# Vinmwaura/Quantized-Autoregression-Image-Generator

Measured on AMD Instinct MI355X. Metric: image-tokens/sec at 1/2/4/8 GPUs; BMU argmin GB/s vs HBM peak, higher is better.
Workload: dtype f32; 1 GPU; BASELINE configs[1]: BMU (K=512; LR patch 32, HR patch 2) + base decoder-only Transformer train step, 32x32x4 latents (128x128 images), 257-token sequences, window 256; batch_per_gpu=64, global_batch=64, seq_len=256, in_dim=512, hidden_dim=2048, heads=64, dec_layers=7, enc_layers=0, params=78226440, parallelism=dp1, launch=eager stream launches

## Files before the change

include/qarig.h:

```cpp
#ifndef QARIG_H
#define QARIG_H

#include <stddef.h>
#include <stdint.h>

#ifdef __cplusplus
extern "C" {
#endif

#define QARIG_OK 0
#define QARIG_ERR_ARG -1
#define QARIG_ERR_LAUNCH -2
#define QARIG_ERR_WORKSPACE -3

#define QARIG_ACT_NONE 0
#define QARIG_ACT_SILU 1
#define QARIG_ACT_TANH 2
#define QARIG_ACT_SIGMOID 3

int qarig_version(void);
const char* qarig_target_arch(void);
int qarig_last_error(char* buf, size_t n);
int qarig_set_option(const char* name, int value);

// ... 129 lines not shown

int qarig_decode_decide(int* ctl, int N, int NB, int beam_width, int draws, float* comb,
                        const int64_t* chunk, float* best_p, int64_t* best_chunk, int* take, void* stream);

int qarig_decode_rows(const int* ctl, float* kv, float* staged, const int* take, int layers2, int N,
                      int NB, int H, int R, int d, int max_len, int restore, void* stream);

int qarig_decode_cache_fill(const float* k, const float* v, int64_t ld, int64_t batch_stride, float* kv,
                            int images, int beams, int H, int d, int P1, int max_len, void* stream);

int qarig_decode_commit(int* ctl, int N, int NB, int beam_width, const int64_t* best_chunk,
                        int64_t* tokens, int64_t ldt, int64_t* ids, void* stream);

int qarig_decode_advance(int* ctl, int beam_width, void* stream);


int qarig_window_step_supported(int R, int window, int D, int H);

int qarig_window_assemble(const int64_t* ring, int64_t ldr, const int* ctl, int R, int W1, int Wp, int D,
                          int V, const float* table, const float* pe, int P, int pos_off, float* x,
                          int* rowmap, int* last_map, int* bad_flag, void* stream);

int qarig_window_attention(const float* q, const float* k, const float* v, int R, int H, int d, int n_keys,
                           int rows, int64_t batch_stride, const float* o_mul, int64_t ldmul, float* o,
                           void* stream);

int qarig_window_append(int* ctl, const int64_t* ids, int64_t* ring, int B, int64_t ldr, int* bad_flag,
                        void* stream);

size_t qarig_colsum_workspace_bytes(int M, int N);
int qarig_colsum_f32(const float* X, int64_t ldx, int M, int N, float* out, int accumulate,
                     void* workspace, size_t ws_bytes, void* stream);


int qarig_patchify_fwd(const float* image, int N, int C, int H, int W, int pH, int pW,
                       float* patches, void* stream);
int qarig_unpatchify_fwd(const float* patches, int N, int C, int H, int W, int pH, int pW,
                         float* image, void* stream);

int qarig_codebook_gather_image(const int64_t* ids, int N, int C, int H, int W, int pH, int pW,
                                const float* codebook, int K, float* image, int* bad_flag,
                                void* stream);

int qarig_gather_rows(const int64_t* ids, int64_t R, int D, int K, const float* table, float* out,
                      int* bad_flag, void* stream);

int qarig_som_weights_fwd(const int64_t* bmu, int64_t R, int K, float two_var, float* g,
                          void* stream);

int qarig_som_band(const float* in, int K, int D, float two_var, int reach, float* out, void* stream);

int qarig_index_histogram(const int64_t* ids, int64_t n, int K, int64_t* counts, int* bad_flag,
                          void* stream);


int qarig_posemb_fwd(const float* pos, int R, int D, const float* freq, float* out, void* stream);

int qarig_assemble_tokens(const int64_t* lr, int S_lr, const int64_t* hr, int S_hr, int N, int base,
                          int k_lr, int k_hr, const int64_t* offs, int W, int64_t* hr_in,
                          int64_t* hr_tg, int64_t* pos, int* bad_flag, void* stream);

int qarig_embedding_fwd(const int64_t* ids, int M, int S, int D, int V, const float* table,
                        const float* pe, float* out, int* bad_flag, void* stream);
int qarig_embedding_bwd(const int64_t* ids, int M, int D, int V, const float* dy, float* dtable,
                        void* stream);

int qarig_layernorm_fwd(const float* x, int M, int D, float eps, const float* gamma,
                        const float* beta, const float* scale, const float* shift,
                        const int* mod_idx, float* y, float* mean, float* rstd, void* stream);
int qarig_layernorm_bwd(const float* dy, const float* x, const float* mean, const float* rstd,
                        const float* gamma, const float* scale, const int* mod_idx, int M, int D,
                        float* dx, float* dy_xhat, const float* dx_add, void* stream);

int qarig_rowmap_build(const int* idx, int M, int P, int* counts, int* offsets, int* rows,
                       int* bad_flag, void* stream);
int qarig_segment_sum(const float* src, const int* offsets, const int* rows, int P, int D,
                      float* out, void* stream);
int qarig_mul_rows_fwd(const float* a, const float* tab, const int* idx, float* y, int M, int D,
                       void* stream);
int qarig_mul_rows_bwd(const float* dy, const float* a, const float* tab, const int* idx, float* da,
                       float* db_tok, int M, int D, void* stream);

int qarig_attention_fwd(const float* q, const float* k, const float* v, int N, int Sq, int Sk,
                        int H, int d, int causal, float sqrt_d, float* o, float* lse,
                        void* stream);
int qarig_attention_bwd(const float* q, const float* k, const float* v, const float* o,
                        const float* dO, const float* lse, int N, int Sq, int Sk, int H, int d,
                        int causal, float sqrt_d, float* dq, float* dk, float* dv, float* delta,
                        void* stream);

int qarig_attention_lp_fwd(const float* q, const float* k, const float* v, int N, int Sq, int Sk, int H,
                           int d, int causal, float sqrt_d, float* o, float* lse, void* stream);
int qarig_attention_lp_bwd(const float* q, const float* k, const float* v, const float* o,
                           const float* dO, const float* lse, int N, int Sq, int Sk, int H, int d,
                           int causal, float sqrt_d, float* dq, float* dk, float* dv, float* delta,
                           void* stream);

int qarig_attention_decode(const float* q, const float* k_new, const float* v_new, float* kcache,
                           float* vcache, int B, int H, int d, int len, const int* len_dev,
                           int max_len, int64_t batch_stride, float sqrt_d, const float* o_mul,
                           float* o, void* stream);

int qarig_cross_entropy_fwd(const float* logits, const int64_t* target, int M, int C, float* loss,
                            float* dlogits, float* row_ws, int* bad_flag, void* stream);

size_t qarig_mse_workspace_bytes(void);
int qarig_mse_fwd(const float* pred, const float* target, int64_t n, float* loss, float* dpred,
                  float* part_ws, void* stream);

int qarig_adam_step(float* p, const float* g, float* m, float* v, int64_t n, float beta1,
                    float beta2, float eps, float step_size, float bc2_sqrt, float grad_scale,
                    const float* dev_step, void* shadow_bf16, void* stream);

int qarig_adam_ema_step(float* p, const float* g, float* m, float* v, float* ema, int64_t n, float beta1,
// ... 50 lines not shown
```

quantized-autoregression-image-generator_amd/csrc/condtable.hip:

```cpp
#include "qarig_common.h"

namespace qarig {

__global__ __launch_bounds__(256) void rowmap_count_kernel(const int* __restrict__ idx, int M, int P,
                                                           int* __restrict__ cnt,
                                                           int* __restrict__ bad) {
    const int p = blockIdx.x;
    int c = 0;
    for (int r = threadIdx.x; r < M; r += 256) {
        const int v = idx[r];
        c += v == p;
        if (p == 0 && (v < 0 || v >= P)) atomicExch(bad, 1);
    }
    __shared__ int part[4];
    c = (int)wave_sum((float)c);
    if ((threadIdx.x & 63) == 0) part[threadIdx.x >> 6] = c;
    __syncthreads();
    if (threadIdx.x == 0) cnt[p] = part[0] + part[1] + part[2] + part[3];
}

__global__ __launch_bounds__(256) void rowmap_scan_kernel(const int* __restrict__ cnt, int P,
                                                          int* __restrict__ offsets) {
    __shared__ int carry;
    __shared__ int buf[256];
// ... 69 lines not shown
            *reinterpret_cast<float4*>(out + (int64_t)p * D + c) = r;
        }
    }
}

__global__ void mul_rows_kernel(const float* __restrict__ a, const float* __restrict__ tab,
                                const int* __restrict__ idx, float* __restrict__ y, int M, int D4) {
    const int64_t total = (int64_t)M * D4;
    for (int64_t i = (int64_t)blockIdx.x * blockDim.x + threadIdx.x; i < total;
         i += (int64_t)gridDim.x * blockDim.x) {
        const int r = (int)(i / D4), c4 = (int)(i - (int64_t)r * D4);
        const float4 av = reinterpret_cast<const float4*>(a)[i];
        const float4 bv = reinterpret_cast<const float4*>(tab)[(int64_t)idx[r] * D4 + c4];
        reinterpret_cast<float4*>(y)[i] = make_float4(av.x * bv.x, av.y * bv.y, av.z * bv.z, av.w * bv.w);
    }
}

__global__ void mul_rows_bwd_kernel(const float* __restrict__ dy, const float* __restrict__ a,
                                    const float* __restrict__ tab, const int* __restrict__ idx,
                                    float* __restrict__ da, float* __restrict__ db_tok, int M,
                                    int D4) {
    const int64_t total = (int64_t)M * D4;
    for (int64_t i = (int64_t)blockIdx.x * blockDim.x + threadIdx.x; i < total;
         i += (int64_t)gridDim.x * blockDim.x) {
        const int r = (int)(i / D4), c4 = (int)(i - (int64_t)r * D4);
        const float4 d = reinterpret_cast<const float4*>(dy)[i];
        const float4 av = reinterpret_cast<const float4*>(a)[i];
        const float4 bv = reinterpret_cast<const float4*>(tab)[(int64_t)idx[r] * D4 + c4];
        reinterpret_cast<float4*>(da)[i] = make_float4(d.x * bv.x, d.y * bv.y, d.z * bv.z, d.w * bv.w);
        reinterpret_cast<float4*>(db_tok)[i] = make_float4(d.x * av.x, d.y * av.y, d.z * av.z, d.w * av.w);
    }
}

}

using namespace qarig;

static dim3 ct_grid(int64_t total) {
    int64_t b = (total + 255) / 256;
    return dim3((unsigned)(b > 8192 ? 8192 : (b < 1 ? 1 : b)));
}

extern "C" int qarig_rowmap_build(const int* idx, int M, int P, int* counts, int* offsets, int* rows,
                                  int* bad_flag, void* stream) {
    QARIG_CHECK_ARG(idx && counts && offsets && rows && bad_flag && M > 0 && P > 0,
                    "rowmap_build: bad arguments");
    QARIG_CHECK_DIMS("rowmap_build", M);
    QARIG_CHECK_DIMS("rowmap_build", P);
    hipStream_t st = (hipStream_t)stream;
    hipLaunchKernelGGL(rowmap_count_kernel, dim3(P), dim3(256), 0, st, idx, M, P, counts, bad_flag);
    QARIG_CHECK_LAUNCH("rowmap count");
    hipLaunchKernelGGL(rowmap_scan_kernel, dim3(1), dim3(256), 0, st, counts, P, offsets);
    QARIG_CHECK_LAUNCH("rowmap scan");
    hipLaunchKernelGGL(rowmap_fill_kernel, dim3(P), dim3(64), 0, st, idx, M, offsets, rows);
    QARIG_CHECK_LAUNCH("rowmap fill");
    return QARIG_OK;
}

extern "C" int qarig_segment_sum(const float* src, const int* offsets, const int* rows, int P, int D,
                                 float* out, void* stream) {
    QARIG_CHECK_ARG(src && offsets && rows && out && P > 0 && D > 0 && D % 4 == 0 &&
                        ((((uintptr_t)src | (uintptr_t)out)) & 15) == 0,
                    "segment_sum: bad arguments (D %% 4 == 0, 16-B aligned)");
    QARIG_CHECK_DIMS("segment_sum", P, D);
    hipLaunchKernelGGL(segment_sum_kernel, dim3(P, (D + 511) / 512), dim3(512), 0,
                       (hipStream_t)stream, src, offsets, rows, D, out);
    QARIG_CHECK_LAUNCH("segment_sum");
    return QARIG_OK;
}

extern "C" int qarig_mul_rows_fwd(const float* a, const float* tab, const int* idx, float* y, int M,
                                  int D, void* stream) {
    QARIG_CHECK_ARG(a && tab && idx && y && M > 0 && D > 0 && D % 4 == 0 &&
                        ((((uintptr_t)a | (uintptr_t)tab | (uintptr_t)y)) & 15) == 0,
                    "mul_rows_fwd: bad arguments (D %% 4 == 0, 16-B aligned)");
    QARIG_CHECK_DIMS("mul_rows_fwd", M, D);
    hipLaunchKernelGGL(mul_rows_kernel, ct_grid((int64_t)M * (D / 4)), dim3(256), 0,
                       (hipStream_t)stream, a, tab, idx, y, M, D / 4);
    QARIG_CHECK_LAUNCH("mul_rows_fwd");
    return QARIG_OK;
}

extern "C" int qarig_mul_rows_bwd(const float* dy, const float* a, const float* tab, const int* idx,
                                  float* da, float* db_tok, int M, int D, void* stream) {
    QARIG_CHECK_ARG(dy && a && tab && idx && da && db_tok && M > 0 && D > 0 && D % 4 == 0 &&
                        ((((uintptr_t)dy | (uintptr_t)a | (uintptr_t)tab | (uintptr_t)da |
                           (uintptr_t)db_tok)) & 15) == 0,
                    "mul_rows_bwd: bad arguments (D %% 4 == 0, 16-B aligned)");
    QARIG_CHECK_DIMS("mul_rows_bwd", M, D);
    hipLaunchKernelGGL(mul_rows_bwd_kernel, ct_grid((int64_t)M * (D / 4)), dim3(256), 0,
                       (hipStream_t)stream, dy, a, tab, idx, da, db_tok, M, D / 4);
    QARIG_CHECK_LAUNCH("mul_rows_bwd");
    return QARIG_OK;
}
```

quantized-autoregression-image-generator_amd/csrc/gemm.hip:

```cpp
#include <stdlib.h>

#include "qarig_common.h"
#include "gemm_epilogue.h"
#include "ring_common.h"

namespace qarig {

struct RowSumHook {
    float rs;
    bool on;
    int tid;
    __device__ __forceinline__ void operator()(const float* ta, const float*) {
        if (on) {
#pragma unroll
            for (int kk = 0; kk < BK; ++kk) rs += ta[kk * LDT + tid];
        }
    }
};

template <class SA, class SB, bool FAST>
__global__ __launch_bounds__(NTHREADS, 2) void gemm_kernel(SA sa, SB sb, GemmEpilogue ep, int M,
                                                           int N, int K, int tiles_n, int splitk,
                                                           float* slabs, int vec_epi) {
    __shared__ __attribute__((aligned(16))) float lds[GEMM_LDS_FLOATS];
// ... 385 lines not shown
__global__ void slab_reduce_kernel(const float* __restrict__ slabs, float* __restrict__ out,
                                   int64_t ldc, int M, int N, int nslab, int accumulate) {
    const int64_t total = (int64_t)M * N;
    for (int64_t i = (int64_t)blockIdx.x * blockDim.x + threadIdx.x; i < total;
         i += (int64_t)gridDim.x * blockDim.x) {
        float s = 0.0f;
        for (int z = 0; z < nslab; ++z) s += slabs[(int64_t)z * total + i];
        const int64_t row = i / N, col = i - row * N;
        out[row * ldc + col] = accumulate ? out[row * ldc + col] + s : s;
    }
}

__global__ void slab_reduce_rowsum_kernel(const float* __restrict__ slabs, float* __restrict__ out,
                                          int64_t ldc, int M, int N, int nslab, int accumulate, int nb,
                                          const float* __restrict__ rs_part, float* __restrict__ rs_out) {
    if ((int)blockIdx.x >= nb) {
        const int m = ((int)blockIdx.x - nb) * blockDim.x + threadIdx.x;
        if (m < M) {
            float s = 0.0f;
            for (int z = 0; z < nslab; ++z) s += rs_part[(int64_t)z * M + m];
            rs_out[m] = accumulate ? rs_out[m] + s : s;
        }
        return;
    }
    const int64_t total = (int64_t)M * N;
    for (int64_t i = (int64_t)blockIdx.x * blockDim.x + threadIdx.x; i < total; i += (int64_t)nb * blockDim.x) {
        float s = 0.0f;
        for (int z = 0; z < nslab; ++z) s += slabs[(int64_t)z * total + i];
        const int64_t row = i / N, col = i - row * N;
        out[row * ldc + col] = accumulate ? out[row * ldc + col] + s : s;
    }
}

__global__ void slab_reduce_epilogue_kernel(const float* __restrict__ slabs, GemmEpilogue ep, int M,
                                            int N, int nslab) {
    const int64_t total = (int64_t)M * N;
    for (int64_t i = (int64_t)blockIdx.x * blockDim.x + threadIdx.x; i < total;
         i += (int64_t)gridDim.x * blockDim.x) {
        float t = 0.0f;
        for (int z = 0; z < nslab; ++z) t += slabs[(int64_t)z * total + i];
        const int64_t row = i / N, col = i - row * N;
        if (ep.bias) t += ep.bias[col];
        if (ep.residual) t += ep.residual[row * ep.ldr + col];
        if (ep.preact) ep.preact[row * ep.ldp + col] = t;
        float y = act_fwd(t, ep.act);
        if (ep.gradz) y *= act_grad(ep.gradz[row * ep.ldz + col], ep.gact);
        ep.C[row * ep.ldc + col] = y;
    }
}

static inline int colsum_rows(int M) { return M >= 32768 ? 512 : (M >= 8192 ? 128 : 32); }
__global__ __launch_bounds__(256) void colsum_partial_kernel(const float* __restrict__ X,
                                                             int64_t ldx, int M, int N,
                                                             float* __restrict__ part, int rows) {
    __shared__ float red[4][64];
    const int cx = threadIdx.x & 63, ry = threadIdx.x >> 6;
    const int col = blockIdx.x * 64 + cx;
    const int r0 = blockIdx.y * rows;
    const int r1 = min(M, r0 + rows);
    float s = 0.0f;
    if (col < N)
        for (int r = r0 + ry; r < r1; r += 4) s += X[(int64_t)r * ldx + col];
    red[ry][cx] = s;
    __syncthreads();
    if (ry == 0 && col < N)
        part[(int64_t)blockIdx.y * N + col] = ((red[0][cx] + red[1][cx]) + red[2][cx]) + red[3][cx];
// ... 303 lines not shown
                               M, N, K, tiles_n, splitk, slabs);
    } else if (pf && fast && vec_epi && !(a_rowsum && a_kcontig) && !(!a_kcontig && b_kcontig)) {
        const int xs = (splitk % 8 == 0 && g_qarig_opt.gemm_xcd_splits != 0) ? 1 : 0;
        const dim3 pgrid = xs ? dim3(grid.x * splitk, 1, 1) : grid;
        if (a_kcontig && b_kcontig)
            hipLaunchKernelGGL((gemm_dma_pf_kernel<true, true>), pgrid, block, 0, st, A, lda, B, ldb, ep, M,
                               N, K, tiles_n, splitk, slabs, xs);
        else if (a_kcontig)
            hipLaunchKernelGGL((gemm_dma_pf_kernel<true, false>), pgrid, block, 0, st, A, lda, B, ldb, ep, M,
                               N, K, tiles_n, splitk, slabs, xs);
        else
            hipLaunchKernelGGL((gemm_dma_pf_kernel<false, false>), pgrid, block, 0, st, A, lda, B, ldb, ep,
                               M, N, K, tiles_n, splitk, slabs, xs);
    } else {
#define QARIG_LAUNCH_GEMM(TA, TB)                                                              \
    do {                                                                                       \
        TA sa{A, lda, M, K, 1.0f, va};                                                         \
        TB sb{B, ldb, N, K, 1.0f, vb};                                                         \
        if (fast)                                                                              \
            hipLaunchKernelGGL((gemm_kernel<TA, TB, true>), grid, block, 0, st, sa, sb, ep, M, \
                               N, K, tiles_n, splitk, slabs, vec_epi);                         \
        else                                                                                   \
            hipLaunchKernelGGL((gemm_kernel<TA, TB, false>), grid, block, 0, st, sa, sb, ep, M,\
                               N, K, tiles_n, splitk, slabs, 0);                               \
    } while (0)
    if (a_kcontig && b_kcontig) QARIG_LAUNCH_GEMM(SrcKContig, SrcKContig);
    else if (a_kcontig && !b_kcontig) QARIG_LAUNCH_GEMM(SrcKContig, SrcXContig);
    else if (!a_kcontig && !b_kcontig) QARIG_LAUNCH_GEMM(SrcXContig, SrcXContig);
    else QARIG_LAUNCH_GEMM(SrcXContig, SrcKContig);
#undef QARIG_LAUNCH_GEMM
    }
    QARIG_CHECK_LAUNCH("gemm");
    if (a_rowsum && splitk > 1 && plain) {
        const int64_t total = (int64_t)M * N;
        int blocks = (int)((total + 255) / 256);
        if (blocks > 2048) blocks = 2048;
        hipLaunchKernelGGL(slab_reduce_rowsum_kernel, dim3(blocks + (M + 255) / 256), dim3(256), 0, st, slabs, C,
                           ldc, M, N, splitk, accumulate, blocks, rs_part, a_rowsum);
        QARIG_CHECK_LAUNCH("gemm slab + rowsum reduce");
        return QARIG_OK;
    }
    if (a_rowsum) {
        hipLaunchKernelGGL(slab_reduce_kernel, dim3((M + 255) / 256), dim3(256), 0, st, rs_part,
                           a_rowsum, (int64_t)M, 1, M, splitk, accumulate);
        QARIG_CHECK_LAUNCH("gemm rowsum reduce");
    }
    if (splitk > 1) {
        const int64_t total = (int64_t)M * N;
        int blocks = (int)((total + 255) / 256);
        if (blocks > 2048) blocks = 2048;
        if (plain)
            hipLaunchKernelGGL(slab_reduce_kernel, dim3(blocks), dim3(256), 0, st, slabs, C, ldc, M, N,
                               splitk, accumulate);
        else
            hipLaunchKernelGGL(slab_reduce_epilogue_kernel, dim3(blocks), dim3(256), 0, st, slabs, ep,
                               M, N, splitk);
        QARIG_CHECK_LAUNCH("gemm slab reduce");
    }
    return QARIG_OK;
}

extern "C" int qarig_slab_reduce_f32(const float* slabs, float* out, int64_t ldc, int M, int N,
                                     int nslab, int accumulate, void* stream) {
    const int64_t total = (int64_t)M * N;
    int blocks = (int)((total + 255) / 256);
    if (blocks > 2048) blocks = 2048;
    hipLaunchKernelGGL(slab_reduce_kernel, dim3(blocks), dim3(256), 0, (hipStream_t)stream, slabs, out,
                       ldc, M, N, nslab, accumulate);
    QARIG_CHECK_LAUNCH("slab reduce");
    return QARIG_OK;
}

extern "C" size_t qarig_colsum_workspace_bytes(int M, int N) {
    if (M < 1 || N < 1 || M > (1 << 30)) return 0;
    const int rows = colsum_rows(M);
    const int chunks = (M + rows - 1) / rows;
    return (size_t)chunks * N * sizeof(float);
}

extern "C" int qarig_colsum_f32(const float* X, int64_t ldx, int M, int N, float* out,
                                int accumulate, void* workspace, size_t ws_bytes, void* stream) {
    QARIG_CHECK_ARG(X && out && M > 0 && N > 0, "colsum: bad arguments");
    QARIG_CHECK_DIMS("colsum", M, N);
    if (!workspace || ws_bytes < qarig_colsum_workspace_bytes(M, N)) {
        qarig_set_error("colsum: workspace too small");
        return QARIG_ERR_WORKSPACE;
    }
    const int rows = colsum_rows(M);
    const int chunks = (M + rows - 1) / rows;
    hipStream_t st = (hipStream_t)stream;
    float* part = (float*)workspace;
    hipLaunchKernelGGL(colsum_partial_kernel, dim3((N + 63) / 64, chunks), dim3(256), 0, st, X, ldx,
                       M, N, part, rows);
    QARIG_CHECK_LAUNCH("colsum partial");
    int blocks = (N + 255) / 256;
    hipLaunchKernelGGL(slab_reduce_kernel, dim3(blocks), dim3(256), 0, st, part, out, (int64_t)N, 1,
                       N, chunks, accumulate);
    QARIG_CHECK_LAUNCH("colsum reduce");
    return QARIG_OK;
}

// ... 171 lines not shown
```

quantized-autoregression-image-generator_amd/qarig/_lib.py:

```python
import ctypes
import os
from ctypes import c_int, c_int64, c_size_t, c_void_p, c_float, c_char_p

import torch

_HERE = os.path.dirname(os.path.abspath(__file__))
LIB_PATH = os.path.join(os.path.dirname(_HERE), "lib",
                        os.environ.get("QARIG_LIB", "libqarig_hip.so"))

P = c_void_p
I = c_int
L = c_int64
Z = c_size_t
F = c_float

SIGNATURES = {
    "qarig_version": (I, []),
    "qarig_target_arch": (c_char_p, []),
    "qarig_last_error": (I, [c_char_p, Z]),
    "qarig_set_option": (I, [c_char_p, I]),
    "qarig_bmu_workspace_bytes": (Z, [L, I]),
    "qarig_bmu_fwd": (I, [P, I, I, I, I, I, I, P, I, I, P, P, Z, P]),
    "qarig_bmu_fwd_prepared": (I, [P, I, I, I, I, I, I, P, I, I, P, P, Z, P, P]),
    "qarig_bmu_fwd_coarse": (I, [P, I, I, I, I, I, I, P, I, I, P, P, P, P]),
# ... 16 lines not shown
                          P]),
    "qarig_gemm_f8_supported": (I, [I, I, I]),
    "qarig_cast_fp8": (I, [P, L, P, P, P, P, P]),
    "qarig_gemm_f8": (I, [P, L, P, L, P, P, P, L, I, I, I, P, P, L, P, L, I, P, L, P, L, P]),
    "qarig_mx_quant_workspace_bytes": (Z, [I, I]),
    "qarig_mx_quant": (I, [P, L, I, I, I, P, P, P, P, P, I, P, Z, P]),
    "qarig_gemm_mx_supported": (I, [I, I, I, I]),
    "qarig_gemm_mx_workspace_bytes": (Z, [I, I, I]),
    "qarig_gemm_mx": (I, [P, L, P, L, P, L, P, L, P, L, I, I, I, P, P, L, P, L, I, P, L, I, I, I, I, P, L, P, L,
                          P, Z, P]),
    "qarig_cast_colsum_workspace_bytes": (Z, [I, I]),
    "qarig_cast_colsum": (I, [P, L, I, I, I, P, P, I, P, Z, P]),
    "qarig_cast_bf16": (I, [P, P, L, P]),
    "qarig_cast_transpose_bf16": (I, [P, L, I, I, P, P]),
    "qarig_colsum_workspace_bytes": (Z, [I, I]),
    "qarig_colsum_f32": (I, [P, L, I, I, P, I, P, Z, P]),
    "qarig_patchify_fwd": (I, [P, I, I, I, I, I, I, P, P]),
    "qarig_unpatchify_fwd": (I, [P, I, I, I, I, I, I, P, P]),
    "qarig_codebook_gather_image": (I, [P, I, I, I, I, I, I, P, I, P, P, P]),
    "qarig_gather_rows": (I, [P, L, I, I, P, P, P, P]),
    "qarig_som_weights_fwd": (I, [P, L, I, F, P, P]),
    "qarig_som_band": (I, [P, I, I, F, I, P, P]),
    "qarig_index_histogram": (I, [P, L, I, P, P, P]),
    "qarig_posemb_fwd": (I, [P, I, I, P, P, P]),
    "qarig_assemble_tokens": (I, [P, I, P, I, I, I, I, I, P, I, P, P, P, P, P]),
    "qarig_embedding_fwd": (I, [P, I, I, I, I, P, P, P, P, P]),
    "qarig_embedding_bwd": (I, [P, I, I, I, P, P, P]),
    "qarig_layernorm_fwd": (I, [P, I, I, F, P, P, P, P, P, P, P, P, P]),
    "qarig_layernorm_bwd": (I, [P, P, P, P, P, P, P, I, I, P, P, P, P]),
    "qarig_rowmap_build": (I, [P, I, I, P, P, P, P, P]),
    "qarig_segment_sum": (I, [P, P, P, I, I, P, P]),
    "qarig_mul_rows_fwd": (I, [P, P, P, P, I, I, P]),
    "qarig_mul_rows_bwd": (I, [P, P, P, P, P, P, I, I, P]),
    "qarig_attention_fwd": (I, [P, P, P, I, I, I, I, I, I, F, P, P, P]),
    "qarig_attention_lp_fwd": (I, [P, P, P, I, I, I, I, I, I, F, P, P, P]),
    "qarig_attention_lp_bwd": (I, [P, P, P, P, P, P, I, I, I, I, I, I, F, P, P, P, P, P]),
    "qarig_attention_decode": (I, [P, P, P, P, P, I, I, I, I, P, I, L, F, P, P, P]),
    "qarig_gemm_grouped_skinny_f32": (I, [P, L, L, P, L, L, P, L, L, P, L, I, I, I, I, I, P]),
    "qarig_gemm_skinny_ln_f32": (I, [P, L, F, P, P, P, P, L, P, L, L, P, L, L, P, L, P, L, I, I, I, I, I, P]),
    "qarig_decode_linear_supported": (I, [I, I, I, I]),
    "qarig_decode_linear_f32": (I, [P, L, L, F, P, P, P, P, L, P, L, L, P, L, P, L, P, L, P, L, L, I, I, I, I, I,
                                    P]),
    "qarig_decode_linear_bf16w": (I, [P, L, L, F, P, P, P, P, L, P, L, L, P, L, P, L, P, L, P, L, L, I, I, I, I, I,
                                      P]),
    "qarig_decode_embed": (I, [P, I, I, I, P, P, P, I, I, P, L, P, P, P, P]),
    "qarig_decode_attention_keys_per_pass": (ctypes.c_uint, [I]),
    "qarig_decode_attention": (I, [P, P, P, P, P, I, I, I, I, P, I, L, L, L, F, P, L, P, P]),
    "qarig_decode_sample": (I, [P, L, I, I, F, I, I, L, P, P, P, I, I, I, I, I, P, P, P, P, P]),
    "qarig_decode_sample_filtered": (I, [P, L, I, I, F, I, I, L, P, P, P, I, I, I, I, I, P, P, P, P, I, F, P]),
    "qarig_decode_decide": (I, [P, I, I, I, I, P, P, P, P, P, P]),
    "qarig_decode_rows": (I, [P, P, P, P, I, I, I, I, I, I, I, I, P]),
    "qarig_decode_cache_fill": (I, [P, P, L, L, P, I, I, I, I, I, I, P]),
    "qarig_decode_commit": (I, [P, I, I, I, P, P, L, P, P]),
    "qarig_decode_advance": (I, [P, I, P]),
    "qarig_window_step_supported": (I, [I, I, I, I]),
    "qarig_window_assemble": (I, [P, L, P, I, I, I, I, I, P, P, I, I, P, P, P, P, P]),
    "qarig_window_attention": (I, [P, P, P, I, I, I, I, I, L, P, L, P, P]),
    "qarig_window_append": (I, [P, P, P, I, L, P, P]),
    "qarig_attention_bwd": (I, [P, P, P, P, P, P, I, I, I, I, I, I, F, P, P, P, P, P]),
    "qarig_cross_entropy_fwd": (I, [P, P, I, I, P, P, P, P, P]),
    "qarig_mse_workspace_bytes": (Z, []),
    "qarig_mse_fwd": (I, [P, P, L, P, P, P, P]),
    "qarig_adam_step": (I, [P, P, P, P, L, F, F, F, F, F, F, P, P, P]),
    "qarig_adam_ema_step": (I, [P, P, P, P, P, L, F, F, F, F, F, F, F, P, P, P]),
    "qarig_swap_f32": (I, [P, P, L, P]),
    "qarig_mul_fwd": (I, [P, P, P, L, P]),
# ... 131 lines not shown
```

quantized-autoregression-image-generator_amd/qarig/functional.py:

```python
import os

import torch

from . import ops
from ._lib import f32c, require_cuda


def _2d(t):
    return t.reshape(-1, t.shape[-1])


FUSED_GRAD_ACCUMULATE = True


def _grad_slot(param):
    if not FUSED_GRAD_ACCUMULATE or not isinstance(param, torch.nn.Parameter):
        return None
    g = param.grad
    if g is None or not g.is_contiguous() or g.dtype != torch.float32 or g.shape != param.shape:
        return None
    return g


def _report_done(param):
# ... 787 lines not shown
        return tuple(grads)

    @staticmethod
    def backward(ctx, *douts):
        if ctx.tiled:
            return _TableProjections._backward_tiled(ctx, douts)
        tab, W = ctx.saved_tensors
        G, D, _ = W.shape
        P = tab.shape[0]
        cols = [f32c(d) if d is not None else torch.zeros((P, D), dtype=torch.float32, device=tab.device)
                for d in douts]
        dcat = torch.cat(cols, dim=1)
        W2 = W.reshape(G * D, D)
        dtab = ops.gemm(dcat, W2, a_kcontig=True, b_kcontig=False) if ctx.needs_input_grad[0] else None
        dW = ops.gemm(dcat, tab, a_kcontig=False, b_kcontig=False,
                      splitk=ops.pick_splitk(G * D, D, P)).reshape(G, D, D)
        db = ops.colsum(dcat).reshape(G, D)
        grads = [dtab]
        wparams, bparams = ctx.params[0::2], ctx.params[1::2]
        wslots = [_grad_slot(p) for p in wparams]
        bslots = [_grad_slot(p) for p in bparams]
        if all(s is not None for s in wslots) and all(s is not None for s in bslots):
            torch._foreach_add_(wslots, list(dW.unbind(0)))
            torch._foreach_add_(bslots, list(db.unbind(0)))
            for p in ctx.params:
                _report_done(p)
            grads += [None] * len(ctx.params)
        else:
            for g in range(G):
                grads += [dW[g], db[g]]
        return tuple(grads)


class _LayerNormModTable(torch.autograd.Function):

    @staticmethod
    def forward(ctx, x, scale_tab, shift_tab, idx, offsets, rows, eps, with_skip=False):
        require_cuda(x, scale_tab, shift_tab)
        x2 = _2d(f32c(x))
        st = f32c(scale_tab)
        y, mean, rstd = ops.layernorm_fwd(x2, scale=st, shift=f32c(shift_tab), eps=eps, mod_idx=idx)
        ctx.save_for_backward(x2, st, mean, rstd, idx, offsets, rows)
        ctx.shape = x.shape
        ctx.set_materialize_grads(False)
        return _with_skip(y.reshape(x.shape), x, with_skip)

    @staticmethod
    def backward(ctx, dy, dskip=None):
        x2, st, mean, rstd, idx, offsets, rows = ctx.saved_tensors
        dy2, add = _skip_grads(dy, dskip, x2)
        dx, dscale_tok = ops.layernorm_bwd(dy2, x2, mean, rstd, scale=st, want_dy_xhat=True,
                                           mod_idx=idx, dx_add=add)
        dscale = ops.segment_sum(dscale_tok, offsets, rows)
        dshift = ops.segment_sum(dy2, offsets, rows)
        return dx.reshape(ctx.shape), dscale, dshift, None, None, None, None, None


def layernorm_mod_table(x, scale_tab, shift_tab, cond, eps=1e-5, with_skip=False):
    if _no_grad():
        require_cuda(x, scale_tab, shift_tab)
        y = ops.layernorm_fwd(_2d(f32c(x)), scale=f32c(scale_tab), shift=f32c(shift_tab), eps=eps,
                              mod_idx=cond.idx)[0].reshape(x.shape)
        return (y, x) if with_skip else y
    return _LayerNormModTable.apply(x, scale_tab, shift_tab, cond.idx, cond.offsets, cond.rows, eps, with_skip)


class _MulTable(torch.autograd.Function):

    @staticmethod
    def forward(ctx, x, gate_tab, idx, offsets, rows):
        require_cuda(x, gate_tab)
        x2 = _2d(f32c(x))
        gt = f32c(gate_tab)
        ctx.save_for_backward(x2, gt, idx, offsets, rows)
        return ops.mul_rows_fwd(x2, gt, idx).reshape(x.shape)

    @staticmethod
    def backward(ctx, dy):
        x2, gt, idx, offsets, rows = ctx.saved_tensors
        dx, dg_tok = ops.mul_rows_bwd(_2d(f32c(dy)), x2, gt, idx)
        return dx.reshape(dy.shape), ops.segment_sum(dg_tok, offsets, rows), None, None, None


def mul_table(x, gate_tab, cond):
    if _no_grad():
        require_cuda(x, gate_tab)
        return ops.mul_rows_fwd(_2d(f32c(x)), f32c(gate_tab), cond.idx).reshape(x.shape)
    return _MulTable.apply(x, gate_tab, cond.idx, cond.offsets, cond.rows)
```

quantized-autoregression-image-generator_amd/qarig/ops.py:

```python
import os

import torch

from . import _lib
from ._lib import check, f32c, ptr, require_cuda, stream, workspace

ACT_IDS = {None: 0, "none": 0, "silu": 1, "tanh": 2, "sigmoid": 3}


def act_id(name):
    if name not in ACT_IDS:
        raise KeyError(name)
    return ACT_IDS[name]


_bmu_images = {}
_bmu_seen = {}
BMU_IMAGE_MIN_ROWS = 24576
BMU_IMAGE_MIN_ROWS_LARGE_K = 2 ** 31 - 1


def bmu_invalidate():
    _bmu_images.clear()
    _bmu_seen.clear()
# ... 853 lines not shown
    rows = torch.empty(M, dtype=torch.int32, device=idx.device)
    check(_lib.load().qarig_rowmap_build(ptr(idx), M, P, ptr(counts), ptr(offsets), ptr(rows),
                                         ptr(_bad_flag(idx.device)), stream()), "qarig_rowmap_build")
    return offsets, rows


def segment_sum(src, offsets, rows):
    P = offsets.numel() - 1
    M, D = src.shape
    assert src.is_contiguous() and rows.numel() == M
    out = torch.empty((P, D), dtype=torch.float32, device=src.device)
    check(_lib.load().qarig_segment_sum(ptr(src), ptr(offsets), ptr(rows), P, D, ptr(out), stream()),
          "qarig_segment_sum")
    return out


def mul_rows_fwd(a, tab, idx):
    M, D = a.shape
    y = torch.empty_like(a)
    check(_lib.load().qarig_mul_rows_fwd(ptr(a), ptr(tab), ptr(idx), ptr(y), M, D, stream()),
          "qarig_mul_rows_fwd")
    return y


def mul_rows_bwd(dy, a, tab, idx):
    M, D = a.shape
    da = torch.empty_like(a)
    db = torch.empty_like(a)
    check(_lib.load().qarig_mul_rows_bwd(ptr(dy), ptr(a), ptr(tab), ptr(idx), ptr(da), ptr(db), M, D,
                                         stream()), "qarig_mul_rows_bwd")
    return da, db


ATTENTION_HEAD_DIMS = (4, 8, 16, 32, 64, 128)
DECODE_HEAD_DIMS = (4, 8, 16, 32, 64, 128)
DECODE_PADDED_HEAD_DIMS = tuple(d for d in range(4, 128, 4) if d not in DECODE_HEAD_DIMS)


def attention_head_dim(d):
    for hd in ATTENTION_HEAD_DIMS:
        if hd >= d:
            return hd
    return None


def attention_fwd(q, k, v, heads, causal, scale_dim=None):
    N, Sq, D = q.shape
    Sk = k.shape[1]
    d = D // heads
    o = torch.empty_like(q)
    lse = torch.empty((N, heads, Sq), dtype=torch.float32, device=q.device)
    lib = _lib.load()
    fn = lib.qarig_attention_lp_fwd if lp_mode() else lib.qarig_attention_fwd
    check(fn(ptr(q), ptr(k), ptr(v), N, Sq, Sk, heads, d, int(causal), float((scale_dim or d) ** 0.5), ptr(o),
             ptr(lse), stream()), "qarig_attention_fwd")
    return o, lse


def attention_decode(q, k_new, v_new, kcache, vcache, length, heads, len_dev=None, o_mul=None, out=None):
    B, D = q.shape
    d = D // heads
    assert kcache.shape == vcache.shape and kcache.shape[0] == B and vcache.stride() == kcache.stride()
    if kcache.dim() == 4:
        assert kcache.shape[1] == heads and kcache.shape[3] == d and kcache.stride(3) == 1 and kcache.stride(2) == d
        max_len, hstride, rstride = kcache.shape[2], kcache.stride(1), d
    else:
# ... 333 lines not shown
```

Before: 291,200 image-tokens/s.

## Fuse table-conditioned LayerNorm/gate backward with segment sums; vectorize split-K slab reduce

Adds per-table-row kernels that compute the LayerNorm-modulation and gate-multiply backward and, in the same pass, accumulate the per-condition dscale/dshift/dgate sums. These replace the two-step path that wrote per-token gradients and then ran segment_sum, which removes one large intermediate tensor write and read. Each block handles one condition row and walks that row's token list with a software-prefetched next row. Separately, the split-K slab reduction gains a float4-vectorized kernel with unrolled slab loads. Parallelism is limited to P blocks, so very few conditions could leave the GPU underused.

```diff
diff --git a/include/qarig.h b/include/qarig.h
--- a/include/qarig.h
+++ b/include/qarig.h
@@ -185,6 +185,9 @@
 int qarig_colsum_f32(const float* X, int64_t ldx, int M, int N, float* out, int accumulate,
                      void* workspace, size_t ws_bytes, void* stream);
 
+int qarig_slab_reduce_rowsum_f32(const float* slabs, float* out, int64_t ldc, int M, int N, int nslab,
+                                 int accumulate, const float* rs_part, float* rs_out, void* stream);
+
 
 int qarig_patchify_fwd(const float* image, int N, int C, int H, int W, int pH, int pW,
                        float* patches, void* stream);
@@ -233,6 +236,12 @@
                        void* stream);
 int qarig_mul_rows_bwd(const float* dy, const float* a, const float* tab, const int* idx, float* da,
                        float* db_tok, int M, int D, void* stream);
+int qarig_layernorm_bwd_table(const float* dy, const float* x, const float* mean, const float* rstd,
+                              const float* scale_tab, const int* offsets, const int* rows, int M, int P,
+                              int D, float* dx, const float* dx_add, float* dscale, float* dshift,
+                              void* stream);
+int qarig_mul_rows_bwd_table(const float* dy, const float* a, const float* tab, const int* offsets,
+                             const int* rows, int M, int P, int D, float* da, float* dg, void* stream);
 
 int qarig_attention_fwd(const float* q, const float* k, const float* v, int N, int Sq, int Sk,
                         int H, int d, int causal, float sqrt_d, float* o, float* lse,
diff --git a/quantized-autoregression-image-generator_amd/csrc/condtable.hip b/quantized-autoregression-image-generator_amd/csrc/condtable.hip
--- a/quantized-autoregression-image-generator_amd/csrc/condtable.hip
+++ b/quantized-autoregression-image-generator_amd/csrc/condtable.hip
@@ -125,6 +125,175 @@
     }
 }
 
+constexpr int TB_WAVES = 2 * SEG_GROUPS;
+
+__device__ __forceinline__ void f4_acc(float4& a, const float4 v) {
+    a.x += v.x; a.y += v.y; a.z += v.z; a.w += v.w;
+}
+
+template <int NV, int NQ>
+__device__ __forceinline__ void table_sums_store(float4 (&part)[NQ][SEG_GROUPS][NV * 64],
+                                                 const float4 (&acc)[NQ][NV], int p, int D,
+                                                 float* const (&out)[NQ]) {
+    const int lane = threadIdx.x & 63, w = threadIdx.x >> 6;
+    if (w >= SEG_GROUPS) {
+#pragma unroll
+        for (int q = 0; q < NQ; ++q)
+#pragma unroll
+            for (int i = 0; i < NV; ++i) part[q][w - SEG_GROUPS][i * 64 + lane] = acc[q][i];
+    }
+    __syncthreads();
+    if (w < SEG_GROUPS) {
+#pragma unroll
+        for (int q = 0; q < NQ; ++q)
+#pragma unroll
+            for (int i = 0; i < NV; ++i) {
+                const float4 a1 = part[q][w][i * 64 + lane], a0 = acc[q][i];
+                part[q][w][i * 64 + lane] = make_float4(a0.x + a1.x, a0.y + a1.y, a0.z + a1.z, a0.w + a1.w);
+            }
+    }
+    __syncthreads();
+    for (int t = threadIdx.x; t < NQ * NV * 64; t += TB_WAVES * 64) {
+        const int q = t / (NV * 64), c = t - q * (NV * 64);
+        float4 r = part[q][0][c];
+#pragma unroll
+        for (int g = 1; g < SEG_GROUPS; ++g) f4_acc(r, part[q][g][c]);
+        *reinterpret_cast<float4*>(out[q] + (int64_t)p * D + c * 4) = r;
+    }
+}
+
+template <int NV>
+__global__ __launch_bounds__(TB_WAVES * 64) void layernorm_bwd_table_kernel(
+    const float* __restrict__ dy, const float* __restrict__ x, const float* __restrict__ mean_in,
+    const float* __restrict__ rstd_in, const float* __restrict__ scale_tab,
+    const int* __restrict__ offsets, const int* __restrict__ rows, int D, float* __restrict__ dx,
+    const float* __restrict__ dx_add, float* __restrict__ dscale, float* __restrict__ dshift) {
+    __shared__ float4 part[2][SEG_GROUPS][NV * 64];
+    const int p = blockIdx.x, lane = threadIdx.x & 63, w = threadIdx.x >> 6;
+    const int beg = offsets[p], end = offsets[p + 1];
+    float4 acc[2][NV];
+    float4 m[NV];
+#pragma unroll
+    for (int i = 0; i < NV; ++i) {
+        acc[0][i] = acc[1][i] = make_float4(0.f, 0.f, 0.f, 0.f);
+        m[i] = *reinterpret_cast<const float4*>(scale_tab + (int64_t)p * D + (i * 64 + lane) * 4);
+    }
+    struct Row {
+        float4 xv[NV], d[NV], a[NV];
+        float mean, rstd;
+    };
+    auto load = [&](Row& t, int row) {
+        const int64_t off = (int64_t)row * D;
+        t.mean = mean_in[row];
+        t.rstd = rstd_in[row];
+#pragma unroll
+        for (int i = 0; i < NV; ++i) {
+            const int c = (i * 64 + lane) * 4;
+            t.xv[i] = *reinterpret_cast<const float4*>(x + off + c);
+            t.d[i] = *reinterpret_cast<const float4*>(dy + off + c);
+            if (dx_add) t.a[i] = *reinterpret_cast<const float4*>(dx_add + off + c);
+        }
+    };
+    int e = beg + (w & (SEG_GROUPS - 1)) + SEG_GROUPS * (w / SEG_GROUPS);
+    int r_cur = e < end ? rows[e] : 0;
+    int r_nxt = e + TB_WAVES < end ? rows[e + TB_WAVES] : 0;
+    Row cur = {};
+    if (e < end) load(cur, r_cur);
+    for (; e < end; e += TB_WAVES) {
+        Row nxt = cur;
+        const int r_nn = e + 2 * TB_WAVES < end ? rows[e + 2 * TB_WAVES] : 0;
+        if (e + TB_WAVES < end) load(nxt, r_nxt);
+        const int64_t off = (int64_t)r_cur * D;
+        const float mean = cur.mean, rstd = cur.rstd;
+        float4 h[NV], g[NV];
+        float s1 = 0.0f, s2 = 0.0f;
+#pragma unroll
+        for (int i = 0; i < NV; ++i) {
+            const float4 xv = cur.xv[i], d = cur.d[i];
+            h[i] = make_float4((xv.x - mean) * rstd, (xv.y - mean) * rstd, (xv.z - mean) * rstd,
+                               (xv.w - mean) * rstd);
+            g[i] = make_float4(d.x * m[i].x, d.y * m[i].y, d.z * m[i].z, d.w * m[i].w);
+            s1 += (g[i].x + g[i].y) + (g[i].z + g[i].w);
+            s2 = fmaf(g[i].x, h[i].x, s2); s2 = fmaf(g[i].y, h[i].y, s2);
+            s2 = fmaf(g[i].z, h[i].z, s2); s2 = fmaf(g[i].w, h[i].w, s2);
+        }
+        s1 = wave_sum(s1) / (float)D;
+        s2 = wave_sum(s2) / (float)D;
+#pragma unroll
+        for (int i = 0; i < NV; ++i) {
+            const int c = (i * 64 + lane) * 4;
+            const float4 d = cur.d[i];
+            float4 r = make_float4(rstd * ((g[i].x - s1) - h[i].x * s2), rstd * ((g[i].y - s1) - h[i].y * s2),
+                                   rstd * ((g[i].z - s1) - h[i].z * s2), rstd * ((g[i].w - s1) - h[i].w * s2));
+            if (dx_add) {
+                const float4 a = cur.a[i];
+                r = make_float4(a.x + r.x, a.y + r.y, a.z + r.z, a.w + r.w);
+            }
+            *reinterpret_cast<float4*>(dx + off + c) = r;
+            f4_acc(acc[0][i], make_float4(d.x * h[i].x, d.y * h[i].y, d.z * h[i].z, d.w * h[i].w));
+            f4_acc(acc[1][i], d);
+        }
+        cur = nxt;
+        r_cur = r_nxt;
+        r_nxt = r_nn;
+    }
+    float* const out[2] = {dscale, dshift};
+    table_sums_store<NV, 2>(part, acc, p, D, out);
+}
+
+template <int NV>
+__global__ __launch_bounds__(TB_WAVES * 64) void mul_rows_bwd_table_kernel(
+    const float* __restrict__ dy, const float* __restrict__ a, const float* __restrict__ tab,
+    const int* __restrict__ offsets, const int* __restrict__ rows, int D, float* __restrict__ da,
+    float* __restrict__ dg) {
+    __shared__ float4 part[1][SEG_GROUPS][NV * 64];
+    const int p = blockIdx.x, lane = threadIdx.x & 63, w = threadIdx.x >> 6;
+    const int beg = offsets[p], end = offsets[p + 1];
+    float4 acc[1][NV];
+    float4 b[NV];
+#pragma unroll
+    for (int i = 0; i < NV; ++i) {
+        acc[0][i] = make_float4(0.f, 0.f, 0.f, 0.f);
+        b[i] = *reinterpret_cast<const float4*>(tab + (int64_t)p * D + (i * 64 + lane) * 4);
+    }
+    struct Row {
+        float4 d[NV], av[NV];
+    };
+    auto load = [&](Row& t, int row) {
+        const int64_t off = (int64_t)row * D;
+#pragma unroll
+        for (int i = 0; i < NV; ++i) {
+            const int c = (i * 64 + lane) * 4;
+            t.d[i] = *reinterpret_cast<const float4*>(dy + off + c);
+            t.av[i] = *reinterpret_cast<const float4*>(a + off + c);
+        }
+    };
+    int e = beg + (w & (SEG_GROUPS - 1)) + SEG_GROUPS * (w / SEG_GROUPS);
+    int r_cur = e < end ? rows[e] : 0;
+    int r_nxt = e + TB_WAVES < end ? rows[e + TB_WAVES] : 0;
+    Row cur = {};
+    if (e < end) load(cur, r_cur);
+    for (; e < end; e += TB_WAVES) {
+        Row nxt = cur;
+        const int r_nn = e + 2 * TB_WAVES < end ? rows[e + 2 * TB_WAVES] : 0;
+        if (e + TB_WAVES < end) load(nxt, r_nxt);
+        const int64_t off = (int64_t)r_cur * D;
+#pragma unroll
+        for (int i = 0; i < NV; ++i) {
+            const int c = (i * 64 + lane) * 4;
+            const float4 d = cur.d[i], av = cur.av[i];
+            *reinterpret_cast<float4*>(da + off + c) =
+                make_float4(d.x * b[i].x, d.y * b[i].y, d.z * b[i].z, d.w * b[i].w);
+            f4_acc(acc[0][i], make_float4(d.x * av.x, d.y * av.y, d.z * av.z, d.w * av.w));
+        }
+        cur = nxt;
+        r_cur = r_nxt;
+        r_nxt = r_nn;
+    }
+    float* const out[1] = {dg};
+    table_sums_store<NV, 1>(part, acc, p, D, out);
+}
+
 }
 
 using namespace qarig;
@@ -186,3 +355,48 @@
     QARIG_CHECK_LAUNCH("mul_rows_bwd");
     return QARIG_OK;
 }
+
+extern "C" int qarig_layernorm_bwd_table(const float* dy, const float* x, const float* mean, const float* rstd,
+                                         const float* scale_tab, const int* offsets, const int* rows, int M, int P,
+                                         int D, float* dx, const float* dx_add, float* dscale, float* dshift,
+                                         void* stream) {
+    QARIG_CHECK_ARG(dy && x && mean && rstd && scale_tab && offsets && rows && dx && dscale && dshift && M > 0 &&
+                        P > 0 && (D == 256 || D == 512 || D == 1024) &&
+                        ((((uintptr_t)dy | (uintptr_t)x | (uintptr_t)scale_tab | (uintptr_t)dx | (uintptr_t)dx_add |
+                           (uintptr_t)dscale | (uintptr_t)dshift)) & 15) == 0,
+                    "layernorm_bwd_table: bad arguments (D = 256, 512 or 1024, 16-B aligned)");
+    QARIG_CHECK_DIMS("layernorm_bwd_table", M, D);
+    QARIG_CHECK_DIMS("layernorm_bwd_table", P, D);
+#define QARIG_LNT_LAUNCH(NV)                                                                                  \
+    hipLaunchKernelGGL((layernorm_bwd_table_kernel<NV>), dim3(P), dim3(TB_WAVES * 64), 0, (hipStream_t)stream, \
+                       dy, x, mean, rstd, scale_tab, offsets, rows, D, dx, dx_add, dscale, dshift)
+    switch (D / 256) {
+        case 1: QARIG_LNT_LAUNCH(1); break;
+        case 2: QARIG_LNT_LAUNCH(2); break;
+        default: QARIG_LNT_LAUNCH(4); break;
+    }
+#undef QARIG_LNT_LAUNCH
+    QARIG_CHECK_LAUNCH("layernorm_bwd_table");
+    return QARIG_OK;
+}
+
+extern "C" int qarig_mul_rows_bwd_table(const float* dy, const float* a, const float* tab, const int* offsets,
+                                        const int* rows, int M, int P, int D, float* da, float* dg, void* stream) {
+    QARIG_CHECK_ARG(dy && a && tab && offsets && rows && da && dg && M > 0 && P > 0 &&
+                        (D == 256 || D == 512 || D == 1024) &&
+                        ((((uintptr_t)dy | (uintptr_t)a | (uintptr_t)tab | (uintptr_t)da | (uintptr_t)dg)) & 15) == 0,
+                    "mul_rows_bwd_table: bad arguments (D = 256, 512 or 1024, 16-B aligned)");
+    QARIG_CHECK_DIMS("mul_rows_bwd_table", M, D);
+    QARIG_CHECK_DIMS("mul_rows_bwd_table", P, D);
+#define QARIG_MRT_LAUNCH(NV)                                                                                 \
+    hipLaunchKernelGGL((mul_rows_bwd_table_kernel<NV>), dim3(P), dim3(TB_WAVES * 64), 0, (hipStream_t)stream, \
+                       dy, a, tab, offsets, rows, D, da, dg)
+    switch (D / 256) {
+        case 1: QARIG_MRT_LAUNCH(1); break;
+        case 2: QARIG_MRT_LAUNCH(2); break;
+        default: QARIG_MRT_LAUNCH(4); break;
+    }
+#undef QARIG_MRT_LAUNCH
+    QARIG_CHECK_LAUNCH("mul_rows_bwd_table");
+    return QARIG_OK;
+}
diff --git a/quantized-autoregression-image-generator_amd/csrc/gemm.hip b/quantized-autoregression-image-generator_amd/csrc/gemm.hip
--- a/quantized-autoregression-image-generator_amd/csrc/gemm.hip
+++ b/quantized-autoregression-image-generator_amd/csrc/gemm.hip
@@ -441,6 +441,80 @@
     }
 }
 
+constexpr int SLAB_UNROLL = 8;
+__global__ __launch_bounds__(256) void slab_reduce_vec_kernel(const float* __restrict__ slabs, float* __restrict__ out,
+                                                              int64_t ldc, int M, int N4, int nslab, int accumulate,
+                                                              int nb, const float* __restrict__ rs_part,
+                                                              float* __restrict__ rs_out) {
+    if ((int)blockIdx.x >= nb) {
+        const int m = ((int)blockIdx.x - nb) * 256 + threadIdx.x;
+        if (m < M) {
+            float s = 0.0f;
+            for (int z0 = 0; z0 < nslab; z0 += 4 * SLAB_UNROLL) {
+                float v[4 * SLAB_UNROLL];
+#pragma unroll
+                for (int j = 0; j < 4 * SLAB_UNROLL; ++j)
+                    if (z0 + j < nslab) v[j] = rs_part[(int64_t)(z0 + j) * M + m];
+#pragma unroll
+                for (int j = 0; j < 4 * SLAB_UNROLL; ++j)
+                    if (z0 + j < nslab) s += v[j];
+            }
+            rs_out[m] = accumulate ? rs_out[m] + s : s;
+        }
+        return;
+    }
+    const int64_t total4 = (int64_t)M * N4;
+    const float4* __restrict__ src = reinterpret_cast<const float4*>(slabs);
+    const int64_t stride = (int64_t)nb * 256;
+    const int64_t srow = stride / N4;
+    const int scol = (int)(stride - srow * N4);
+    int64_t i = (int64_t)blockIdx.x * 256 + threadIdx.x;
+    int64_t row = i / N4;
+    int col = (int)(i - row * N4);
+    for (; i < total4; i += stride) {
+        float4* dst = reinterpret_cast<float4*>(out + row * ldc) + col;
+        float4 s = make_float4(0.f, 0.f, 0.f, 0.f);
+        for (int z0 = 0; z0 < nslab; z0 += SLAB_UNROLL) {
+            float4 v[SLAB_UNROLL];
+#pragma unroll
+            for (int j = 0; j < SLAB_UNROLL; ++j)
+                if (z0 + j < nslab) v[j] = src[(int64_t)(z0 + j) * total4 + i];
+#pragma unroll
+            for (int j = 0; j < SLAB_UNROLL; ++j)
+                if (z0 + j < nslab) { s.x += v[j].x; s.y += v[j].y; s.z += v[j].z; s.w += v[j].w; }
+        }
+        if (accumulate) {
+            const float4 o = *dst;
+            s = make_float4(o.x + s.x, o.y + s.y, o.z + s.z, o.w + s.w);
+        }
+        *dst = s;
+        row += srow;
+        col += scol;
+        if (col >= N4) { col -= N4; ++row; }
+    }
+}
+
+static void launch_slab_reduce(hipStream_t st, const float* slabs, float* out, int64_t ldc, int M, int N, int nslab,
+                               int accumulate, const float* rs_part, float* rs_out) {
+    const int64_t total = (int64_t)M * N;
+    const int rs_blocks = rs_part ? (M + 255) / 256 : 0;
+    if (N % 4 == 0 && ldc % 4 == 0 && ((((uintptr_t)slabs | (uintptr_t)out)) & 15) == 0) {
+        int blocks = (int)((total / 4 + 255) / 256);
+        if (blocks > 2048) blocks = 2048;
+        hipLaunchKernelGGL(slab_reduce_vec_kernel, dim3(blocks + rs_blocks), dim3(256), 0, st, slabs, out, ldc, M,
+                           N / 4, nslab, accumulate, blocks, rs_part, rs_out);
+        return;
+    }
+    int blocks = (int)((total + 255) / 256);
+    if (blocks > 2048) blocks = 2048;
+    if (rs_part)
+        hipLaunchKernelGGL(slab_reduce_rowsum_kernel, dim3(blocks + rs_blocks), dim3(256), 0, st, slabs, out, ldc, M,
+                           N, nslab, accumulate, blocks, rs_part, rs_out);
+    else
+        hipLaunchKernelGGL(slab_reduce_kernel, dim3(blocks), dim3(256), 0, st, slabs, out, ldc, M, N, nslab,
+                           accumulate);
+}
+
 __global__ void slab_reduce_epilogue_kernel(const float* __restrict__ slabs, GemmEpilogue ep, int M,
                                             int N, int nslab) {
     const int64_t total = (int64_t)M * N;
@@ -810,11 +884,7 @@
     }
     QARIG_CHECK_LAUNCH("gemm");
     if (a_rowsum && splitk > 1 && plain) {
-        const int64_t total = (int64_t)M * N;
-        int blocks = (int)((total + 255) / 256);
-        if (blocks > 2048) blocks = 2048;
-        hipLaunchKernelGGL(slab_reduce_rowsum_kernel, dim3(blocks + (M + 255) / 256), dim3(256), 0, st, slabs, C,
-                           ldc, M, N, splitk, accumulate, blocks, rs_part, a_rowsum);
+        launch_slab_reduce(st, slabs, C, ldc, M, N, splitk, accumulate, rs_part, a_rowsum);
         QARIG_CHECK_LAUNCH("gemm slab + rowsum reduce");
         return QARIG_OK;
     }
@@ -824,15 +894,15 @@
         QARIG_CHECK_LAUNCH("gemm rowsum reduce");
     }
     if (splitk > 1) {
-        const int64_t total = (int64_t)M * N;
-        int blocks = (int)((total + 255) / 256);
-        if (blocks > 2048) blocks = 2048;
-        if (plain)
-            hipLaunchKernelGGL(slab_reduce_kernel, dim3(blocks), dim3(256), 0, st, slabs, C, ldc, M, N,
-                               splitk, accumulate);
-        else
+        if (plain) {
+            launch_slab_reduce(st, slabs, C, ldc, M, N, splitk, accumulate, nullptr, nullptr);
+        } else {
+            const int64_t total = (int64_t)M * N;
+            int blocks = (int)((total + 255) / 256);
+            if (blocks > 2048) blocks = 2048;
             hipLaunchKernelGGL(slab_reduce_epilogue_kernel, dim3(blocks), dim3(256), 0, st, slabs, ep,
                                M, N, splitk);
+        }
         QARIG_CHECK_LAUNCH("gemm slab reduce");
     }
     return QARIG_OK;
@@ -840,11 +910,18 @@
 
 extern "C" int qarig_slab_reduce_f32(const float* slabs, float* out, int64_t ldc, int M, int N,
                                      int nslab, int accumulate, void* stream) {
-    const int64_t total = (int64_t)M * N;
-    int blocks = (int)((total + 255) / 256);
-    if (blocks > 2048) blocks = 2048;
-    hipLaunchKernelGGL(slab_reduce_kernel, dim3(blocks), dim3(256), 0, (hipStream_t)stream, slabs, out,
-                       ldc, M, N, nslab, accumulate);
+    launch_slab_reduce((hipStream_t)stream, slabs, out, ldc, M, N, nslab, accumulate, nullptr, nullptr);
+    QARIG_CHECK_LAUNCH("slab reduce");
+    return QARIG_OK;
+}
+
+extern "C" int qarig_slab_reduce_rowsum_f32(const float* slabs, float* out, int64_t ldc, int M, int N, int nslab,
+                                            int accumulate, const float* rs_part, float* rs_out, void* stream) {
+    QARIG_CHECK_ARG(slabs && out && nslab > 0 && nslab <= 4096 && ldc >= N && (rs_part == nullptr) == (rs_out == nullptr),
+                    "slab_reduce_rowsum: bad arguments");
+    QARIG_CHECK_DIMS("slab_reduce_rowsum", M, N);
+    QARIG_CHECK_DIMS("slab_reduce_rowsum", M, ldc);
+    launch_slab_reduce((hipStream_t)stream, slabs, out, ldc, M, N, nslab, accumulate, rs_part, rs_out);
     QARIG_CHECK_LAUNCH("slab reduce");
     return QARIG_OK;
 }
diff --git a/quantized-autoregression-image-generator_amd/qarig/_lib.py b/quantized-autoregression-image-generator_amd/qarig/_lib.py
--- a/quantized-autoregression-image-generator_amd/qarig/_lib.py
+++ b/quantized-autoregression-image-generator_amd/qarig/_lib.py
@@ -72,6 +72,9 @@
     "qarig_segment_sum": (I, [P, P, P, I, I, P, P]),
     "qarig_mul_rows_fwd": (I, [P, P, P, P, I, I, P]),
     "qarig_mul_rows_bwd": (I, [P, P, P, P, P, P, I, I, P]),
+    "qarig_layernorm_bwd_table": (I, [P, P, P, P, P, P, P, I, I, I, P, P, P, P, P]),
+    "qarig_mul_rows_bwd_table": (I, [P, P, P, P, P, I, I, I, P, P, P]),
+    "qarig_slab_reduce_rowsum_f32": (I, [P, P, L, I, I, I, I, P, P, P]),
     "qarig_attention_fwd": (I, [P, P, P, I, I, I, I, I, I, F, P, P, P]),
     "qarig_attention_lp_fwd": (I, [P, P, P, I, I, I, I, I, I, F, P, P, P]),
     "qarig_attention_lp_bwd": (I, [P, P, P, P, P, P, I, I, I, I, I, I, F, P, P, P, P, P]),
diff --git a/quantized-autoregression-image-generator_amd/qarig/functional.py b/quantized-autoregression-image-generator_amd/qarig/functional.py
--- a/quantized-autoregression-image-generator_amd/qarig/functional.py
+++ b/quantized-autoregression-image-generator_amd/qarig/functional.py
@@ -843,6 +843,9 @@
         return tuple(grads)
 
 
+TABLE_BWD_CALLS = {"fused": 0, "two_step": 0}
+
+
 class _LayerNormModTable(torch.autograd.Function):
 
     @staticmethod
@@ -860,6 +863,12 @@
     def backward(ctx, dy, dskip=None):
         x2, st, mean, rstd, idx, offsets, rows = ctx.saved_tensors
         dy2, add = _skip_grads(dy, dskip, x2)
+        M, D = x2.shape
+        if ops.table_bwd_fused(M, st.shape[0], D, dy2, x2, st, add):
+            TABLE_BWD_CALLS["fused"] += 1
+            dx, dscale, dshift = ops.layernorm_bwd_table(dy2, x2, mean, rstd, st, offsets, rows, dx_add=add)
+            return dx.reshape(ctx.shape), dscale, dshift, None, None, None, None, None
+        TABLE_BWD_CALLS["two_step"] += 1
         dx, dscale_tok = ops.layernorm_bwd(dy2, x2, mean, rstd, scale=st, want_dy_xhat=True,
                                            mod_idx=idx, dx_add=add)
         dscale = ops.segment_sum(dscale_tok, offsets, rows)
@@ -889,7 +898,13 @@
     @staticmethod
     def backward(ctx, dy):
         x2, gt, idx, offsets, rows = ctx.saved_tensors
-        dx, dg_tok = ops.mul_rows_bwd(_2d(f32c(dy)), x2, gt, idx)
+        dy2 = _2d(f32c(dy))
+        if ops.table_bwd_fused(x2.shape[0], gt.shape[0], x2.shape[1], dy2, x2, gt):
+            TABLE_BWD_CALLS["fused"] += 1
+            dx, dg = ops.mul_rows_bwd_table(dy2, x2, gt, offsets, rows)
+            return dx.reshape(dy.shape), dg, None, None, None
+        TABLE_BWD_CALLS["two_step"] += 1
+        dx, dg_tok = ops.mul_rows_bwd(dy2, x2, gt, idx)
         return dx.reshape(dy.shape), ops.segment_sum(dg_tok, offsets, rows), None, None, None
 
 
diff --git a/quantized-autoregression-image-generator_amd/qarig/ops.py b/quantized-autoregression-image-generator_amd/qarig/ops.py
--- a/quantized-autoregression-image-generator_amd/qarig/ops.py
+++ b/quantized-autoregression-image-generator_amd/qarig/ops.py
@@ -909,6 +909,55 @@
     return da, db
 
 
+TABLE_BWD_MIN_TOKENS_PER_ROW = 2
+TABLE_BWD_WIDTHS = (256, 512, 1024)
+
+
+def table_bwd_fused(M, P, D, *tensors):
+    return (D in TABLE_BWD_WIDTHS and M >= TABLE_BWD_MIN_TOKENS_PER_ROW * P
+            and all(t is None or t.data_ptr() % 16 == 0 for t in tensors))
+
+
+def layernorm_bwd_table(dy, x2d, mean, rstd, scale_tab, offsets, rows, dx_add=None):
+    M, D = x2d.shape
+    P = offsets.numel() - 1
+    assert dy.shape == x2d.shape and dy.is_contiguous() and x2d.is_contiguous() and rows.numel() == M
+    assert scale_tab.shape == (P, D) and scale_tab.is_contiguous()
+    if dx_add is not None:
+        assert dx_add.shape == x2d.shape and dx_add.dtype == torch.float32 and dx_add.is_contiguous()
+    dx = torch.empty_like(x2d)
+    dscale = torch.empty((P, D), dtype=torch.float32, device=x2d.device)
+    dshift = torch.empty((P, D), dtype=torch.float32, device=x2d.device)
+    check(_lib.load().qarig_layernorm_bwd_table(ptr(dy), ptr(x2d), ptr(mean), ptr(rstd), ptr(scale_tab),
+                                                ptr(offsets), ptr(rows), M, P, D, ptr(dx), ptr(dx_add),
+                                                ptr(dscale), ptr(dshift), stream()), "qarig_layernorm_bwd_table")
+    return dx, dscale, dshift
+
+
+def mul_rows_bwd_table(dy, a, tab, offsets, rows):
+    M, D = a.shape
+    P = offsets.numel() - 1
+    assert dy.shape == a.shape and dy.is_contiguous() and a.is_contiguous() and rows.numel() == M
+    assert tab.shape == (P, D) and tab.is_contiguous()
+    da = torch.empty_like(a)
+    dg = torch.empty((P, D), dtype=torch.float32, device=a.device)
+    check(_lib.load().qarig_mul_rows_bwd_table(ptr(dy), ptr(a), ptr(tab), ptr(offsets), ptr(rows), M, P, D,
+                                               ptr(da), ptr(dg), stream()), "qarig_mul_rows_bwd_table")
+    return da, dg
+
+
+def slab_reduce(slabs, out, M, N, accumulate=False, rs_part=None, rs_out=None):
+    nslab = slabs.shape[0]
+    assert slabs.is_contiguous() and slabs.dtype == torch.float32 and slabs.shape[1:] == (M, N)
+    assert out.dtype == torch.float32 and out.stride(1) == 1 and out.shape[0] >= M and out.shape[1] >= N
+    if rs_part is not None:
+        assert rs_part.is_contiguous() and rs_part.shape == (nslab, M) and rs_out.is_contiguous()
+    check(_lib.load().qarig_slab_reduce_rowsum_f32(ptr(slabs), ptr(out), out.stride(0), M, N, nslab,
+                                                   int(accumulate), ptr(rs_part), ptr(rs_out), stream()),
+          "qarig_slab_reduce_rowsum_f32")
+    return out
+
+
 ATTENTION_HEAD_DIMS = (4, 8, 16, 32, 64, 128)
 DECODE_HEAD_DIMS = (4, 8, 16, 32, 64, 128)
 DECODE_PADDED_HEAD_DIMS = tuple(d for d in range(4, 128, 4) if d not in DECODE_HEAD_DIMS)
```

Measured after the change: 294,900 image-tokens/s (median of 6 runs). 1.3% higher.
